# ChainSafe/lumenos

Hardware: AMD Instinct MI355X
Metric: prove_eval_seconds_16384x4096 (lower is better)
Workload: dtype u64; 1 GPU; Encode+Commit+InnerProduct(r,b)+QueryCols 16384x4096 LogN=14 L=12 K=2 rhoInv=2 queries=309; parallelism=1 GPU: the whole job resident in HBM

## Files before the change

### lumenos_amd/csrc/lm_keyswitch.hip

```cpp
#include <cstdlib>
#include <cstring>

#include "lm_ks_host.h"

static uint32_t ks_batch(const lumen_ctx *ctx) { return ctx->tune.ks_batch; }

__device__ __forceinline__ u32 bx_v(u128 A, u128 M, u64 y0, u64 y1, u64 m0, u64 m1) {
    const u128 D1 = A >= M ? A - M : M - A, D2 = 2 * M - A;
    if ((u64)(D1 >> 64) >= 8 && (u64)(D2 >> 64) >= 8) return A >= M ? 1u : 0u;
    double vf = 0.0;
    vf += (double)y0 / (double)m0;
    vf += (double)y1 / (double)m1;
    return (u32)(u64)vf;
}

__device__ __forceinline__ void pack_pair(u64 a, u64 b, u64 m0, u64 m1, u128 M, u64 &hi, u64 &lo) {
    u64 l1, h1, l2, h2;
    mul128(a, m1, l1, h1);
    mul128(b, m0, l2, h2);
    const u128 A = (((u128)h1 << 64) | l1) + (((u128)h2 << 64) | l2);
    const u32 v = bx_v(A, M, a, b, m0, m1);
    const u128 W = A + (v == 0 ? 2 * M : (v == 1 ? M : (u128)0));
    hi = (u64)(W >> LM_W_SPLIT), lo = (u64)W & ((1ull << LM_W_SPLIT) - 1);
}

__global__ __launch_bounds__(256) void k_pack_v(u64 *__restrict__ y, size_t poly_stride, uint32_t npoly,
                                                uint32_t ngroups, uint32_t group_limbs, uint32_t first_mod,
                                                uint32_t nlimbs_total, uint32_t logN, lm_mods mods) {
    const uint32_t N = 1u << logN;
    const size_t total = (size_t)npoly * ngroups * (N / 2), stride = (size_t)gridDim.x * blockDim.x;
    for (size_t g = (size_t)blockIdx.x * blockDim.x + threadIdx.x; g < total; g += stride) {
        const uint32_t i = (uint32_t)(g & (N / 2 - 1)) * 2;
        const uint32_t grp = (uint32_t)((g >> (logN - 1)) % ngroups), p = (uint32_t)((g >> (logN - 1)) / ngroups);
        const uint32_t l0 = grp * group_limbs;
        if (l0 + 1 >= nlimbs_total) continue;
        u64 *y0 = y + (size_t)p * poly_stride + (size_t)l0 * N + i;
        const ulonglong2 av = *reinterpret_cast<const ulonglong2 *>(y0);
        const ulonglong2 bv = *reinterpret_cast<const ulonglong2 *>(y0 + N);
        const u64 m0 = mods.m[first_mod + l0].q, m1 = mods.m[first_mod + l0 + 1].q;
        u64 Ml, Mh;
        mul128(m0, m1, Ml, Mh);
        const u128 M = ((u128)Mh << 64) | Ml;
        ulonglong2 hv, lv;
#pragma unroll
        for (int e = 0; e < 2; e++) {
            const u64 a = e ? av.y : av.x, b = e ? bv.y : bv.x;
            u64 hi, lo;
            pack_pair(a, b, m0, m1, M, hi, lo);
            if (e) hv.y = hi, lv.y = lo;
            else hv.x = hi, lv.x = lo;
        }
        *reinterpret_cast<ulonglong2 *>(y0) = hv;
        *reinterpret_cast<ulonglong2 *>(y0 + N) = lv;
    }
}

template <int LOGN>
__global__ LM_GEOM_BOUNDS(lm_geom_lds(LOGN)) void k_intt_pack(const u64 *__restrict__ acc, u64 *coef, uint32_t B,
                                                                  uint32_t L, uint32_t nf, lm_mods mods,
                                                                  lm_ninv_t yscale, const tw_t *__restrict__ tw_all) {
    extern __shared__ __attribute__((aligned(16))) u64 sm[];
    constexpr uint32_t N = 1u << LOGN;
    const uint32_t tid = threadIdx.x;
    if (blockIdx.x >= B * nf) {
        const uint32_t k = blockIdx.x - B * nf, l = 2 * nf + k / B, b = k % B;
        const u64 *p = acc + (((size_t)b * 2 + 1) * L + l) * N;
        u64 *o = coef + ((size_t)b * L + l) * N;
        const lm_qc q = lm_make_qc(mods.m[l]);
        const tw_t sc = yscale.t[l];
        auto ld = [&](uint32_t i0, u64 *v, int count) { lm_load_run(p, i0, v, count); };
        auto st = [&](uint32_t i, u64 v) { o[i] = lm_shoup_cs(v, sc, q.q, q.nq); };
        lm_ntt_inverse<LOGN>(sm, tw_all + (size_t)l * N, q, tid, ld, st);
        return;
    }
    const uint32_t d = blockIdx.x / B, b = blockIdx.x % B;
    const uint32_t l0 = 2 * d, l1 = l0 + 1;
    const u64 *c1 = acc + ((size_t)b * 2 + 1) * L * N;
    u64 *o0 = coef + ((size_t)b * L + l0) * N;
    const lm_qc q0 = lm_make_qc(mods.m[l0]);
    const tw_t s0 = yscale.t[l0];
    {
        const u64 *p = c1 + (size_t)l0 * N;
        auto ld = [&](uint32_t i0, u64 *v, int count) { lm_load_run(p, i0, v, count); };
        auto st = [&](uint32_t i, u64 v) { o0[i] = lm_shoup_cs(v, s0, q0.q, q0.nq); };
        lm_ntt_inverse<LOGN>(sm, tw_all + (size_t)l0 * N, q0, tid, ld, st);
    }
    __syncthreads();
    {
        const lm_qc q1 = lm_make_qc(mods.m[l1]);
        const tw_t s1 = yscale.t[l1];
        const u64 *p = c1 + (size_t)l1 * N;
        u64 Ml, Mh;
        mul128(q0.q, q1.q, Ml, Mh);
        auto uni = [](u64 x) {
            return (u64)(uint32_t)__builtin_amdgcn_readfirstlane((int)(uint32_t)x) |
                   (u64)(uint32_t)__builtin_amdgcn_readfirstlane((int)(uint32_t)(x >> 32)) << 32;
        };
        const u128 M = ((u128)uni(Mh) << 64) | uni(Ml);
        auto ld = [&](uint32_t i0, u64 *v, int count) { lm_load_run(p, i0, v, count); };
        constexpr int R_LAST = lm_pass_r(LOGN, 0), LOG_T0 = LOGN - R_LAST;
        constexpr int PF = (1 << R_LAST) * 5 / 8;
        struct pack_t {
            u64 *o0;
            const lm_qc &q0, &q1;
            tw_t s1;
            u128 M;
            u64 y0[PF];
            __device__ __forceinline__ void pre(uint32_t w) {
#pragma unroll
                for (int k = 0; k < PF; k++) y0[k] = o0[w + ((uint32_t)k << LOG_T0)];
            }
            __device__ __forceinline__ void operator()(uint32_t i, u64 v, int k) {
                const u64 y1 = lm_shoup_cs(v, s1, q1.q, q1.nq);
                uint32_t j = i;
                asm volatile("" : "+v"(j));
                const u64 a = k < PF ? y0[k < PF ? k : 0] : o0[j];
                u64 hi, lo;
                pack_pair(a, y1, q0.q, q1.q, M, hi, lo);
                o0[j] = hi, o0[j + N] = lo;
                if (k >= PF && (k & 1)) asm volatile("" ::: "memory");
            }
        } st{o0, q0, q1, s1, M, {}};
        uint32_t tid1 = tid;
        asm volatile("" : "+v"(tid1));
        lm_ntt_inverse<LOGN>(sm, tw_all + (size_t)l1 * N, q1, tid1, ld, st);
    }
}

template <int LOGN>
__global__ LM_GEOM_BOUNDS(lm_geom_fwd(LOGN)) void k_modup_ntt(const u64 *__restrict__ coef, const u64 *__restrict__ acc,
                                                    u64 *__restrict__ ext, const bx_t *__restrict__ bx,
                                                    uint32_t B, uint32_t L, uint32_t K, uint32_t beta,
                                                    const uint32_t *__restrict__ work, lm_mods mods,
                                                    const tw_t *__restrict__ tw_all) {
    extern __shared__ __attribute__((aligned(16))) u64 sm[];
    constexpr uint32_t N = 1u << LOGN;
    const uint32_t tid = threadIdx.x, LK = L + K;
    const uint32_t wk = work[blockIdx.x];
    const uint32_t b = wk & 0xFFFF, d = (wk >> 16) & 0xFF, t = wk >> 24;
    const bx_t c = bx[d * LK + t];
    u64 *o = ext + ks_ext_at(b, d, t, B, beta) * N;
    const lm_qc qc = lm_make_qc(mods.m[t]);
    const u64 *s0 = coef + ((size_t)b * L + d * K) * N;
    const u64 *s1 = c.ns == 2 ? s0 + N : s0;
    auto ld = [&](uint32_t i) { return bx_apply(c, s0[i], s1[i], qc); };
    auto out = [&](uint32_t j, u64 v0, u64 v1) {
        ulonglong2 y;
        y.x = v0, y.y = v1;
        *reinterpret_cast<ulonglong2 *>(o + j) = y;
    };
    if constexpr (LOGN == 14) {
        lm_w14_runs st{sm};
        auto after = [&](uint32_t i0, uint32_t) { lm_w14_linear_out(sm, tid, i0, out); };
        lm_ntt_forward_w14(sm, tw_all + (size_t)t * N, qc, tid, ld, st, after);
    } else {
        lm_lds_runs st{sm};
        auto after = [&](uint32_t, uint32_t) { lm_linear_out<LOGN>(sm, tid, out); };
        lm_ntt_forward<LOGN>(sm, tw_all + (size_t)t * N, qc, tid, ld, st, after);
    }
}

#ifndef LM_MAC_COLS
#define LM_MAC_COLS 4
#endif
#ifndef LM_MAC_VEC
#define LM_MAC_VEC 1
#endif
#ifndef LM_MAC_PREFETCH
#define LM_MAC_PREFETCH 1
#endif
template <int VEC>
struct mac_vec;
template <>
struct mac_vec<1> {
    u64 v[1];
    static __device__ __forceinline__ mac_vec load(const u64 *p) { return mac_vec{{*p}}; }
    static __device__ __forceinline__ mac_vec load_once(const u64 *p) { return mac_vec{{__builtin_nontemporal_load(p)}}; }
    __device__ __forceinline__ void store(u64 *p) const { *p = v[0]; }
};
template <>
struct mac_vec<2> {
    u64 v[2];
    static __device__ __forceinline__ mac_vec load(const u64 *p) {
        const ulonglong2 a = *reinterpret_cast<const ulonglong2 *>(p);
        return mac_vec{{a.x, a.y}};
    }
    static __device__ __forceinline__ mac_vec load_once(const u64 *p) {
        return mac_vec{{__builtin_nontemporal_load(p), __builtin_nontemporal_load(p + 1)}};
    }
    __device__ __forceinline__ void store(u64 *p) const {
        ulonglong2 a;
        a.x = v[0], a.y = v[1];
        *reinterpret_cast<ulonglong2 *>(p) = a;
    }
};
struct mac_acc {
    u64 a0, a1, a3;
    u32 c0, c1;
    __device__ __forceinline__ void clear() { a0 = a1 = a3 = 0, c0 = c1 = 0; }
    __device__ __forceinline__ void value(u64 &lo, u64 &hi) const {
        lo = a0 + (a1 << 32);
        hi = a3 + c0 + (a1 >> 32) + ((u64)c1 << 32) + (lo < a0 ? 1 : 0);
    }
};
__device__ __forceinline__ void mac2(mac_acc &p, mac_acc &q, u64 x, u64 k0, u64 k1) {
    const u32 x0 = (u32)x, x1 = (u32)(x >> 32);
#if LM_ASM_SHOUP
    asm("v_mad_u64_u32 %[pa0], s[98:99], %[x0], %[k00], %[pa0]\n\t"
// ... 282 lines not shown
    out->d_bxp = tb->d_bxp.get();
    out->d_pinv = tb->d_pinv.get();
    out->yscale = &tb->yscale;
    return 0;
}

int lm_launch_pack_v(lumen_ctx *ctx, u64 *y, size_t poly_stride, uint32_t npoly, uint32_t ngroups,
                     uint32_t group_limbs, uint32_t first_mod, uint32_t nlimbs_total) {
    hipLaunchKernelGGL(k_pack_v, dim3(2048), dim3(256), 0, ctx->stream, y, poly_stride, npoly, ngroups, group_limbs,
                       first_mod, nlimbs_total, ctx->logN, ctx->mods);
    LM_HIP(ctx, hipGetLastError());
    return 0;
}

namespace {

static int interleave_work_lists(lumen_ctx *ctx, const std::vector<std::vector<uint32_t>> &lists, size_t expect,
                                 const char *what, std::map<uint32_t, lm_dev<uint32_t>> &cache, uint32_t cache_key,
                                 const uint32_t **out) {
    std::vector<uint32_t> order;
    order.reserve(expect);
    std::vector<size_t> pos(8, 0);
    for (bool any = true; any;) {
        any = false;
        for (uint32_t x = 0; x < 8; x++)
            if (pos[x] < lists[x].size()) {
                order.push_back(lists[x][pos[x]++]);
                any = true;
            }
    }
    LM_CHECK(ctx, order.size() == expect, "%s work list is inconsistent", what);
    lm_dev<uint32_t> d;
    if (int rc = d.upload(ctx, order, "a key-switch work list")) return rc;
    *out = (cache[cache_key] = std::move(d)).get();
    return 0;
}

static int modup_work_list(lumen_ctx *ctx, KsTables *tb, uint32_t B, const uint32_t **out) {
    const uint32_t LM_MODUP_TGROUP = ctx->tune.modup_tgroup;
    LM_SHARED_LOCK(ctx);
    LM_CHECK(ctx, B >= 1 && B <= 65535 && tb->beta <= 255 && ctx->L + ctx->K <= 255,
             "key-switch batch of %u columns (beta %u) does not fit the packed work list", B, tb->beta);
    const uint32_t cache_key = B | (LM_MODUP_TGROUP << 16);
    auto it = tb->d_work.find(cache_key);
    if (it != tb->d_work.end()) {
        *out = it->second.get();
        return 0;
    }
    const uint32_t LK = ctx->L + ctx->K, beta = tb->beta;
    std::vector<std::vector<uint8_t>> need(beta);
    for (uint16_t pr : tb->pairs) need[pr & 0xFF].push_back((uint8_t)(pr >> 8));
    std::vector<std::vector<uint32_t>> lists(8);
    for (uint32_t x = 0; x < 8; x++)
        for (uint32_t t0 = 0; t0 < LK; t0 += LM_MODUP_TGROUP)
            for (uint32_t b = x; b < B; b += 8)
                for (uint32_t d = 0; d < beta; d++)
                    for (uint8_t t : need[d])
                        if (t >= t0 && t < t0 + LM_MODUP_TGROUP) lists[x].push_back(b | (d << 16) | ((uint32_t)t << 24));
    return interleave_work_lists(ctx, lists, (size_t)B * tb->pairs.size(), "extension", tb->d_work, cache_key, out);
}

static int moddown_work_list(lumen_ctx *ctx, KsTables *tb, uint32_t B, const uint32_t **out) {
    const uint32_t LM_MODDOWN_TGROUP = ctx->tune.moddown_tgroup;
    LM_SHARED_LOCK(ctx);
    LM_CHECK(ctx, B >= 1 && 2 * (uint64_t)B <= 65535, "key-switch batch of %u columns does not fit the packed work list", B);
    const uint32_t cache_key = B | (LM_MODDOWN_TGROUP << 17);
    auto it = tb->d_work_down.find(cache_key);
    if (it != tb->d_work_down.end()) {
        *out = it->second.get();
        return 0;
    }
    const uint32_t L = ctx->L;
    std::vector<std::vector<uint32_t>> lists(8);
    for (uint32_t x = 0; x < 8; x++)
        for (uint32_t t0 = 0; t0 < L; t0 += LM_MODDOWN_TGROUP)
            for (uint32_t pw = x; pw < 2 * B; pw += 8)
                for (uint32_t t = t0; t < std::min<uint32_t>(t0 + LM_MODDOWN_TGROUP, L); t++) lists[x].push_back(pw | (t << 16));
    return interleave_work_lists(ctx, lists, (size_t)2 * B * L, "ModDown", tb->d_work_down, cache_key, out);
}

static uint32_t ks_lanes(const lumen_ctx *ctx) {
    return ctx->tune.ks_lanes ? ctx->tune.ks_lanes : (ctx->logN <= 13 ? 2 : 1);
}
template <int LOGN>
static uint32_t intt_pack_slots(lumen_ctx *ctx) {
    static const uint32_t v = [&] {
        hipDeviceProp_t prop;
        int per_cu = 0;
        if (hipGetDeviceProperties(&prop, ctx->device) != hipSuccess) return 256u;
        (void)hipFuncSetAttribute(reinterpret_cast<const void *>(&k_intt_pack<LOGN>),
                                  hipFuncAttributeMaxDynamicSharedMemorySize, 160 * 1024);
        constexpr lm_geom g = lm_geom_lds(LOGN);
        if (hipOccupancyMaxActiveBlocksPerMultiprocessor(&per_cu, k_intt_pack<LOGN>, g.threads, g.lds) != hipSuccess || per_cu < 1) {
            per_cu = (int)std::max<size_t>(1, std::min<size_t>(160 * 1024 / g.lds, 2048 / g.threads));
        }
        (void)hipGetLastError();
        if (ctx->tune.debug)
            fprintf(stderr, "[lumenos_hip] k_intt_pack<%d>: %d workgroup(s) per CU, %d CUs\n", LOGN, per_cu,
                    prop.multiProcessorCount);
        return (uint32_t)prop.multiProcessorCount * (uint32_t)per_cu;
    }();
    return v;
}
static uint32_t ks_fused_digits(lumen_ctx *ctx, uint32_t B, uint32_t L) {
    const long forced = ctx->tune.ks_fused_digits;
    const uint32_t pairs = L / 2;
    if (forced >= 0) return std::min<uint32_t>((uint32_t)forced, pairs);
    uint32_t slots = 0;
    if (lm_for_logn(ctx, ctx->logN, [&](auto n) { return slots = intt_pack_slots<n>(ctx), 0; })) return 0;
    for (uint32_t nf = pairs; nf >= 1; nf--)
        if (((uint64_t)B * nf) % slots == 0) return nf;
    return 0;
}

struct LaneGuard {
    lumen_ctx *ctx;
    hipStream_t saved;
    LaneGuard(lumen_ctx *c, int lane) : ctx(c), saved(c->stream) {
        if (lane) ctx->stream = ctx->stream2;
    }
    ~LaneGuard() { ctx->stream = saved; }
};

static dim3 ks_mac_grid(const lumen_ctx *ctx, uint32_t B) {
    return dim3(((ctx->N / LM_MAC_VEC + 255) / 256) * (ctx->L + ctx->K) * ((B + LM_MAC_COLS - 1) / LM_MAC_COLS));
}

}

int rotate_accumulate(lumen_ctx *ctx, const u64 *acc, u64 *acc_out, uint32_t B, const lm_galois_key &gk,
                      KsTables *tb, const KsScratch &s) {
    const uint32_t N = ctx->N, L = ctx->L, K = ctx->K, beta = tb->beta;
    const uint32_t nf = K == 2 ? ks_fused_digits(ctx, B, L) : 0;
    if (nf) {
        const uint32_t grid = B * nf + B * (L - 2 * nf);
        lm_prof_scope ps(ctx, "ks_intt_c1", (uint64_t)B * L);
        if (int rc = lm_for_logn(ctx, ctx->logN, [&](auto n) {
                return lm_launch(ctx, k_intt_pack<n>, lm_geom_lds(n), grid, acc, s.coef, B, L, nf, ctx->mods, tb->yscale,
                                 ctx->sh->tw_inv.get());
            }))
            return rc;
    } else {
        if (int rc = lm_launch_ntt_strided(ctx, acc + (size_t)L * N, (size_t)2 * L * N, s.coef, (size_t)L * N, B,
                                           lm_map_q(L), true, "ks_intt_c1", &tb->yscale))
            return rc;
    }
    if (K == 2 && nf < beta) {
        lm_prof_scope ps(ctx, "ks_pack_v", (uint64_t)B);
        hipLaunchKernelGGL(k_pack_v, dim3(2048), dim3(256), 0, ctx->stream, s.coef + (size_t)2 * nf * N, (size_t)L * N,
                           B, beta - nf, K, 2 * nf, L - 2 * nf, ctx->logN, ctx->mods);
        LM_HIP(ctx, hipGetLastError());
    }
    {
        const uint64_t nb = (uint64_t)B * tb->pairs.size();
        const uint32_t *work = nullptr;
        if (int rc = modup_work_list(ctx, tb, B, &work)) return rc;
        lm_prof_scope ps(ctx, "ks_modup_ntt", nb);
        if (int rc = lm_for_logn(ctx, ctx->logN, [&](auto n) {
                return lm_launch(ctx, k_modup_ntt<n>, lm_geom_fwd(n), (uint32_t)nb, s.coef, acc, s.ext, tb->d_bx.get(), B, L, K, beta,
                                 work, ctx->mods, ctx->sh->tw_fwd.get());
            }))
            return rc;
    }
    {
        lm_prof_scope ps(ctx, "ks_mac", (uint64_t)B);
        hipLaunchKernelGGL(k_ks_mac, ks_mac_grid(ctx, B), dim3(256), 0, ctx->stream, s.ext, acc, gk.d_key.get(), s.u, B, L, K,
                           beta, ctx->logN, ctx->mods);
        LM_HIP(ctx, hipGetLastError());
    }
    {
        u64 *up = s.u + ks_u_at(0, L, B, L, K) * N;
        const size_t pstride = (size_t)K * N;
        if (int rc = lm_launch_ntt_strided(ctx, up, pstride, up, pstride, B * 2, lm_map_p(ctx), true, "ks_intt_p",
                                           &tb->yscale))
            return rc;
        if (K == 2) {
            lm_prof_scope ps(ctx, "ks_pack_v", (uint64_t)B);
            hipLaunchKernelGGL(k_pack_v, dim3(2048), dim3(256), 0, ctx->stream, up, pstride, B * 2, 1u, K, L, K,
                               ctx->logN, ctx->mods);
            LM_HIP(ctx, hipGetLastError());
        }
    }
    {
        const uint32_t *work_down = nullptr;
        if (int rc = moddown_work_list(ctx, tb, B, &work_down)) return rc;
        lm_prof_scope ps(ctx, "ks_moddown_ntt", (uint64_t)B * 2 * L);
        return lm_for_logn(ctx, ctx->logN, [&](auto n) {
            return lm_launch(ctx, k_moddown_ntt<n>, lm_geom_lds(n), B * 2 * L, s.u, acc, acc_out, tb->d_bxp.get(), tb->d_pinv.get(),
                             gk.d_index.get(), gk.d_inv_index.get(), work_down, B, L, K, ctx->mods, ctx->sh->tw_fwd.get());
        });
    }
}

namespace {

int inner_sum_batch(lumen_ctx *ctx, u64 *acc, uint32_t B, uint32_t n, KsTables *tb, const KsScratch &s) {
    uint64_t gal[64];
    const uint32_t cnt = lumen_inner_sum_galois_elements(ctx, n, gal);
    for (uint32_t r = 0; r < cnt; r++) {
        const lm_galois_key *gk;
        {
            LM_SHARED_LOCK(ctx);
            auto it = ctx->gkeys.find(gal[r]);
            LM_CHECK(ctx, it != ctx->gkeys.end(), "Galois key for element %llu not loaded",
                     (unsigned long long)gal[r]);
            gk = &it->second;
        }
        u64 *src = (r & 1) ? s.acc2 : acc, *dst = (r & 1) ? acc : s.acc2;
        if (int rc = rotate_accumulate(ctx, src, dst, B, *gk, tb, s)) return rc;
    }
    if (cnt & 1)
        LM_HIP(ctx, hipMemcpyAsync(acc, s.acc2, (size_t)B * 2 * ctx->L * ctx->N * 8, hipMemcpyDeviceToDevice,
                                   ctx->stream));
    return 0;
}

}

extern "C" int lumen_ks_mac_probe(lumen_ctx *ctx, uint32_t batch, const void *ext, const void *acc, const void *key,
                                  void *u, uint32_t reps, float *ms_per_launch) {
    LM_CHECK(nullptr, ctx && ms_per_launch, "lumen_ks_mac_probe: NULL argument");
// ... 122 lines not shown
```

### lumenos_amd/csrc/lm_ntt.hip

```cpp
#include "lm_ntt_dev.h"

template <int LOGN, bool INV>
constexpr lm_geom k_limb_ntt_geom = INV ? lm_geom_lds(LOGN) : lm_geom_fwd(LOGN);
template <int LOGN, bool INV>
__global__ LM_GEOM_BOUNDS((k_limb_ntt_geom<LOGN, INV>)) void k_limb_ntt(const u64 *src, size_t src_poly_stride, u64 *dst,
                                                   size_t dst_poly_stride, uint32_t npoly, lm_modmap map,
                                                   lm_mods mods, lm_ninv_t ninv,
                                                   const tw_t *__restrict__ tw_all) {
    extern __shared__ __attribute__((aligned(16))) u64 sm[];
    constexpr uint32_t N = 1u << LOGN;
    const uint32_t tid = threadIdx.x;
    const uint32_t limb = blockIdx.x / npoly, poly = blockIdx.x % npoly;
    const uint32_t mi = map.idx[limb];
    const lm_qc c = lm_make_qc(mods.m[mi]);
    const u64 *p = src + (size_t)poly * src_poly_stride + (size_t)limb * N;
    u64 *o = dst + (size_t)poly * dst_poly_stride + (size_t)limb * N;
    const tw_t *tw = tw_all + (size_t)mi * N;
    if (INV) {
        const tw_t ni = ninv.t[mi];
        auto st = [&](uint32_t i, u64 v) { o[i] = lm_shoup_cs(v, ni, c.q, c.nq); };
        auto ld = [&](uint32_t i0, u64 *v, int count) { lm_load_run(p, i0, v, count); };
        lm_ntt_inverse<LOGN>(sm, tw, c, tid, ld, st);
    } else {
        auto ld = [&](uint32_t i) { return p[i]; };
        auto st = [&](uint32_t i0, const u64 *v, int count) {
            u64 r[8];
#pragma unroll
            for (int k = 0; k < 8; k++)
                if (k < count) r[k] = lm_reduce_s(v[k], c.q, c.nq, c.qinv64);
            lm_store_run(o, i0, r, count);
        };
        if constexpr (LOGN == 14)
            lm_ntt_forward_w14(sm, tw, c, tid, ld, st);
        else
            lm_ntt_forward<LOGN>(sm, tw, c, tid, ld, st);
    }
}

static int launch_limb_ntt(lumen_ctx *ctx, uint32_t logn, bool inverse, uint32_t grid, const u64 *src,
                           size_t src_poly_stride, u64 *dst, size_t dst_poly_stride, uint32_t npoly,
                           const lm_modmap &map, const lm_mods &mods, const lm_ninv_t &ninv, const tw_t *tw) {
    return lm_for_logn(ctx, logn, [&](auto n) {
        if (inverse)
            return lm_launch(ctx, k_limb_ntt<n, true>, k_limb_ntt_geom<n, true>, grid, src, src_poly_stride, dst,
                             dst_poly_stride, npoly, map, mods, ninv, tw);
        return lm_launch(ctx, k_limb_ntt<n, false>, k_limb_ntt_geom<n, false>, grid, src, src_poly_stride, dst,
                         dst_poly_stride, npoly, map, mods, ninv, tw);
    });
}

int lm_launch_ntt_subring(lumen_ctx *ctx, uint32_t logn, const tw_t *tw, tw_t ninv_scale, const u64 *src,
                          size_t src_poly_stride, u64 *dst, size_t dst_poly_stride, uint32_t npoly,
                          uint32_t mod_idx, bool inverse, const mod_t *explicit_mod) {
    if (!npoly) return 0;
    lm_modmap map = lm_map_q(1);
    map.idx[0] = 0;
    lm_mods mods = ctx->mods;
    mods.m[0] = explicit_mod ? *explicit_mod : ctx->mods.m[mod_idx];
    lm_ninv_t ninv = lm_ninv_of(ctx);
    ninv.t[0] = ninv_scale;
    return launch_limb_ntt(ctx, logn, inverse, npoly, src, src_poly_stride, dst, dst_poly_stride, npoly, map, mods, ninv, tw);
}

int lm_launch_ntt_strided(lumen_ctx *ctx, const u64 *src, size_t src_poly_stride, u64 *dst,
                          size_t dst_poly_stride, uint32_t npoly, const lm_modmap &map, bool inverse,
                          const char *prof_name, const lm_ninv_t *inv_scale) {
    if (!npoly || !map.period) return 0;
    const lm_ninv_t ninv = inv_scale ? *inv_scale : lm_ninv_of(ctx);
    const uint64_t nblocks64 = (uint64_t)npoly * map.period;
    LM_CHECK(ctx, nblocks64 < (1ull << 31), "NTT grid too large: %llu", (unsigned long long)nblocks64);
    lm_prof_scope ps(ctx, prof_name ? prof_name : (inverse ? "limb_intt" : "limb_ntt"), nblocks64);
    return launch_limb_ntt(ctx, ctx->logN, inverse, (uint32_t)nblocks64, src, src_poly_stride, dst, dst_poly_stride, npoly,
                           map, ctx->mods, ninv, inverse ? ctx->sh->tw_inv.get() : ctx->sh->tw_fwd.get());
}

int lm_launch_ntt(lumen_ctx *ctx, u64 *d, uint32_t npoly, const lm_modmap &map, bool inverse) {
    const size_t stride = (size_t)map.period * ctx->N;
    return lm_launch_ntt_strided(ctx, d, stride, d, stride, npoly, map, inverse, nullptr, nullptr);
}

extern "C" int lumen_set_ntt(lumen_ctx *ctx, lumen_set *set, int inverse) {
    LM_CHECK(nullptr, ctx && set, "lumen_set_ntt: NULL argument");
    LM_ENTER(ctx);
    LM_FULL_WIDTH(ctx, set, "lumen_set_ntt");
    return lm_launch_ntt(ctx, set->d, set->count * 2, lm_map_q(set->nl), inverse != 0);
}
```

### lumenos_amd/csrc/lm_ntt_dev.h

```cpp
#pragma once
#include <cstring>
#include <type_traits>
#include <utility>

#include "lm_common.h"

#define LM_PAD(i) ((i) + ((i) >> 3))
template <int LOG_STRIDE>
__device__ __forceinline__ uint32_t lm_pad_at(uint32_t base, uint32_t pbase, int k) {
    if constexpr (LOG_STRIDE >= 3)
        return pbase + (uint32_t)k * ((1u << LOG_STRIDE) + (1u << (LOG_STRIDE - 3)));
    else
        return LM_PAD(base + ((uint32_t)k << LOG_STRIDE));
}
#define LM_MAX_PASSES 8

struct lm_ninv_t {
    tw_t t[LM_MAX_LIMBS];
};

__host__ __device__ constexpr int lm_ilog2(int x) { return x <= 1 ? 0 : 1 + lm_ilog2(x >> 1); }
__host__ __device__ constexpr size_t lm_lds_for(uint32_t n) { return (size_t)(n + (n >> 3) + 2) * sizeof(u64); }
struct lm_geom {
    int threads;
// ... 648 lines not shown
#ifndef LM_INV_TW_PREFETCH
#define LM_INV_TW_PREFETCH 1
#endif
template <int LOGN, int R, int LT>
__device__ __forceinline__ void lm_inv_mid(u64 *s, const tw_t *tw, const lm_qc &c, uint32_t tid) {
    using D = lm_deal<LOGN, R>;
    if (!D::valid(tid)) return;
    constexpr bool UW = LT >= 6;
    lm_inv_twset<R, UW, false> T[2];
    T[0].load(tw, LOGN, LT, D::local(tid, 0) >> LT);
#pragma unroll
    for (uint32_t m = 0; m < D::reps; m++) {
        const uint32_t w = D::local(tid, m);
        const uint32_t blk = w >> LT, off = w & ((1u << LT) - 1);
        const uint32_t base = (blk << (LT + R)) + off;
        u64 e[1 << R];
        const uint32_t pb = LM_PAD(base);
#pragma unroll
        for (int k = 0; k < (1 << R); k++) e[k] = s[lm_pad_at<LT>(base, pb, k)];
        if (LM_INV_TW_PREFETCH && m + 1 < D::reps) T[(m + 1) & 1].load(tw, LOGN, LT, D::local(tid, m + 1) >> LT);
        if (!LM_INV_TW_PREFETCH && m) T[0].load(tw, LOGN, LT, blk);
        lm_inv_stages<R, UW, false, false>(e, T[LM_INV_TW_PREFETCH ? (m & 1) : 0], c);
#pragma unroll
        for (int k = 0; k < (1 << R); k++) s[lm_pad_at<LT>(base, pb, k)] = e[k];
    }
}

template <class S, class = void>
struct lm_has_slot : std::false_type {};
template <class S>
struct lm_has_slot<S, std::void_t<decltype(std::declval<S &>()(0u, (u64)0, 0))>> : std::true_type {};

template <int LOGN, int R, class Storer>
__device__ __forceinline__ void lm_inv_last(const u64 *s, const tw_t *tw, const lm_qc &c, uint32_t tid, Storer &st) {
    constexpr uint32_t log_t0 = LOGN - R, items = 1u << log_t0, NT = lm_nthreads(LOGN);
    constexpr uint32_t reps = items / NT ? items / NT : 1;
    lm_inv_twset<R, true, false> T;
    T.load(tw, LOGN, log_t0, 0);
#pragma unroll 1
    for (uint32_t m = 0; m < reps; m++) {
        const uint32_t w = tid + m * NT;
        if (items < NT && w >= items) break;
        u64 e[1 << R];
#pragma unroll
        for (int k = 0; k < (1 << R); k++) e[k] = s[lm_pad_at<log_t0>(w, LM_PAD(w), k)];
        if constexpr (lm_has_pre<Storer>::value) st.pre(w);
        lm_inv_stages<R, true, true, false>(e, T, c);
#pragma unroll
        for (int k = 0; k < (1 << R); k++) {
            if constexpr (lm_has_slot<Storer>::value)
                st(w + ((uint32_t)k << log_t0), e[k], k);
            else
                st(w + ((uint32_t)k << log_t0), e[k]);
        }
    }
}

template <int LOGN, int P, int LT, class Loader, class Storer>
__device__ __forceinline__ void lm_inv_rec(u64 *sm, const tw_t *tw, const lm_qc &c, uint32_t tid, Loader &ld,
                                           Storer &st) {
    constexpr int NP = lm_npasses(LOGN), R = lm_pass_r(LOGN, NP - 1 - P);
    constexpr bool cross = lm_cross_r(LOGN) > 0;
    if constexpr (P == 0)
        lm_inv_first<LOGN, R>(sm, tw, c, tid, ld);
    else if constexpr (P == NP - 1)
        lm_inv_last<LOGN, R>(sm, tw, c, tid, st);
    else
        lm_inv_mid<LOGN, R, LT>(sm, tw, c, tid);
    if constexpr (P + 1 < NP) {
        if constexpr (P + 2 == NP && cross)
            __syncthreads();
        else
            lm_wave_sync();
        lm_inv_rec<LOGN, P + 1, LT + R>(sm, tw, c, tid, ld, st);
    }
}
template <int LOGN, class Loader, class Storer>
__device__ __forceinline__ void lm_ntt_inverse(u64 *sm, const tw_t *tw, const lm_qc &c, uint32_t tid, Loader &ld,
                                               Storer &st) {
    static_assert(lm_npasses(LOGN) >= 2, "a transform needs a loading and a storing pass");
    lm_inv_rec<LOGN, 0, 0>(sm, tw, c, tid, ld, st);
}

__device__ __forceinline__ void lm_load_run(const u64 *p, uint32_t i0, u64 *v, int count) {
    if (count == 2) {
        const ulonglong2 a = *reinterpret_cast<const ulonglong2 *>(p + i0);
        v[0] = a.x, v[1] = a.y;
    } else {
#pragma unroll
        for (int k = 0; k < 8; k += 2) {
            if (k < count) {
                const ulonglong2 a = *reinterpret_cast<const ulonglong2 *>(p + i0 + k);
                v[k] = a.x, v[k + 1] = a.y;
            }
        }
    }
}
struct lm_lds_runs {
    u64 *sm;
    __device__ __forceinline__ void operator()(uint32_t i0, const u64 *v, int count) const {
#pragma unroll
        for (int k = 0; k < 8; k++)
            if (k < count) sm[LM_PAD(i0 + k)] = v[k];
    }
};
template <int LOGN, class F>
__device__ __forceinline__ void lm_linear_out(const u64 *sm, uint32_t tid, F f) {
    constexpr uint32_t NW = lm_nthreads(LOGN) / 64, BLK = (1u << LOGN) / NW, IT = BLK / 128 ? BLK / 128 : 1;
    const uint32_t wave = tid >> 6, lane = tid & 63;
    lm_wave_sync();
#pragma unroll
    for (uint32_t k = 0; k < IT; k++) {
        const uint32_t j = wave * BLK + 2 * lane + k * 128;
        if (BLK >= 128 || 2 * lane < BLK) f(j, sm[LM_PAD(j)], sm[LM_PAD(j + 1)]);
    }
}

__device__ __forceinline__ void lm_store_run(u64 *p, uint32_t i0, const u64 *v, int count) {
#pragma unroll
    for (int k = 0; k < 8; k += 2) {
        if (k < count) {
            ulonglong2 a;
            a.x = v[k], a.y = v[k + 1];
            *reinterpret_cast<ulonglong2 *>(p + i0 + k) = a;
        }
    }
}
```

### lumenos_amd/csrc/lm_rescale.hip

```cpp
#include "lm_ntt_dev.h"

struct rescale_consts {
    u64 half;
    u64 half_mod[LM_MAX_LIMBS];
    tw_t qlinv[LM_MAX_LIMBS];
};

template <int LOGN>
__global__ LM_GEOM_BOUNDS(lm_geom_lds(LOGN)) void k_rescale_last(const u64 *__restrict__ src, size_t src_poly_stride,
                                                       uint32_t last, u64 *__restrict__ tbuf, mod_t md,
                                                       tw_t ninv, u64 half, const tw_t *__restrict__ tw) {
    extern __shared__ __attribute__((aligned(16))) u64 sm[];
    constexpr uint32_t N = 1u << LOGN;
    const uint32_t tid = threadIdx.x;
    const lm_qc c = lm_make_qc(md);
    const u64 *p = src + (size_t)blockIdx.x * src_poly_stride + (size_t)last * N;
    u64 *o = tbuf + (size_t)blockIdx.x * N;
    auto ld = [&](uint32_t i0, u64 *v, int count) { lm_load_run(p, i0, v, count); };
    auto st = [&](uint32_t i, u64 v) { o[i] = lm_addmod(lm_shoup_cs(v, ninv, c.q, c.nq), half, c.q); };
    lm_ntt_inverse<LOGN>(sm, tw, c, tid, ld, st);
}

template <int LOGN>
__global__ LM_GEOM_BOUNDS(lm_geom_lds(LOGN)) void k_rescale_limb(const u64 *src, size_t src_poly_stride, u64 *dst,
                                                       size_t dst_poly_stride, const u64 *__restrict__ tbuf,
                                                       uint32_t npoly, lm_mods mods, rescale_consts rc,
                                                       const tw_t *__restrict__ tw_all) {
    extern __shared__ __attribute__((aligned(16))) u64 sm[];
    constexpr uint32_t N = 1u << LOGN;
    const uint32_t tid = threadIdx.x;
    const uint32_t limb = blockIdx.x / npoly, poly = blockIdx.x % npoly;
    const lm_qc c = lm_make_qc(mods.m[limb]);
    const u64 hm = rc.half_mod[limb];
    const tw_t qlinv = rc.qlinv[limb];
    const u64 *t = tbuf + (size_t)poly * N;
    const u64 *cin = src + (size_t)poly * src_poly_stride + (size_t)limb * N;
    u64 *o = dst + (size_t)poly * dst_poly_stride + (size_t)limb * N;
    auto ld = [&](uint32_t i) { return lm_submod(lm_reduce_s(t[i], c.q, c.nq, c.qinv64), hm, c.q); };
    auto st = [&](uint32_t i0, const u64 *v, int count) {
        u64 cv[8], r[8];
        lm_load_run(cin, i0, cv, count);
#pragma unroll
        for (int k = 0; k < 8; k++)
            if (k < count) r[k] = lm_shoup_cs(lm_submod(cv[k], lm_reduce_s(v[k], c.q, c.nq, c.qinv64), c.q), qlinv, c.q, c.nq);
        lm_store_run(o, i0, r, count);
    };
    lm_ntt_forward<LOGN>(sm, tw_all + (size_t)limb * N, c, tid, ld, st);
}

struct rs_step_t {
    u64 k;
    u64 pad;
    tw_t inv;
};
struct rs_half_t {
    u64 h[LM_MAX_LIMBS];
};
struct RescaleTables {
    lm_dev<rs_step_t> d_steps;
    rs_half_t half;
};

static int get_rescale_tables(lumen_ctx *ctx, RescaleTables **out) {
    LM_SHARED_LOCK(ctx);
    auto it = ctx->ext.find("rescale_tables");
    if (it != ctx->ext.end()) {
        *out = static_cast<RescaleTables *>(it->second.get());
        return 0;
    }
    auto sp = std::make_shared<RescaleTables>();
    std::vector<rs_step_t> steps((size_t)LM_MAX_LIMBS * LM_MAX_LIMBS);
    memset(steps.data(), 0, steps.size() * sizeof(rs_step_t));
    for (uint32_t l = 0; l < LM_MAX_LIMBS; l++) {
        const uint64_t ql = ctx->mod[l < ctx->L ? l : 0], half = (ql - 1) >> 1;
        sp->half.h[l] = half;
        for (uint32_t j = 0; j < l && l < ctx->L; j++) {
            const uint64_t qj = ctx->mod[j];
            rs_step_t &e = steps[(size_t)l * LM_MAX_LIMBS + j];
            const uint64_t M = ql / qj + 1;
            if (M > 16) return 2;
            e.k = half + M * qj;
            e.inv = h_tw(h_invmod(ql % qj, qj), qj);
        }
    }
    if (int rc = sp->d_steps.upload(ctx, steps, "the rescale tables")) return rc;
    ctx->ext["rescale_tables"] = sp;
    *out = sp.get();
    return 0;
}

__global__ __launch_bounds__(256) void k_rescale_coef(const u64 *__restrict__ coef, size_t src_poly_stride,
                                                      u64 *__restrict__ dst, size_t dst_poly_stride, uint32_t nl,
                                                      uint32_t target, uint32_t logN, size_t total, lm_mods mods,
                                                      const rs_step_t *__restrict__ steps, rs_half_t half) {
    const size_t idx = (size_t)blockIdx.x * blockDim.x + threadIdx.x;
    if (idx >= total) return;
    const size_t poly = idx >> logN, i = idx & (((size_t)1 << logN) - 1);
    const u64 *p = coef + poly * src_poly_stride + i;
    u64 c[LM_MAX_LIMBS];
#pragma unroll
    for (int j = 0; j < LM_MAX_LIMBS; j++) c[j] = (uint32_t)j < nl ? p[(size_t)j << logN] : 0;
#pragma unroll
    for (int l = LM_MAX_LIMBS - 1; l >= 1; l--) {
        if ((uint32_t)l < nl && (uint32_t)l >= target) {
            const u64 ql = mods.m[l].q;
            u64 t = lm_csub(lm_csub(c[l], 2 * ql), ql);
            t = lm_addmod(t, half.h[l], ql);
#pragma unroll
            for (int j = 0; j < l; j++) {
                const rs_step_t e = steps[l * LM_MAX_LIMBS + j];
                c[j] = lm_shoup3<true>(c[j] + e.k - t, e.inv.w, e.inv.wp, 0 - mods.m[j].q);
            }
        }
    }
    u64 *o = dst + poly * dst_poly_stride + i;
#pragma unroll
    for (int j = 0; j < LM_MAX_LIMBS; j++)
        if ((uint32_t)j < target) {
            const u64 qj = mods.m[j].q;
            o[(size_t)j << logN] = lm_csub(lm_csub(c[j], 2 * qj), qj);
        }
}

static int rescale_polys_coef(lumen_ctx *ctx, const u64 *src, uint32_t nl, u64 *dst, uint32_t target, uint32_t npoly,
                              u64 *work) {
    RescaleTables *tb = nullptr;
    if (int rc = get_rescale_tables(ctx, &tb)) return rc;
    const uint32_t N = ctx->N;
    if (int rc = lm_launch_ntt_strided(ctx, src, (size_t)nl * N, work, (size_t)nl * N, npoly, lm_map_q(nl), true,
                                       "rescale_intt", nullptr))
        return rc;
    {
        lm_prof_scope ps(ctx, "rescale_coef", npoly);
        const size_t total = (size_t)npoly * N;
        hipLaunchKernelGGL(k_rescale_coef, dim3((uint32_t)((total + 255) / 256)), dim3(256), 0, ctx->stream, work,
                           (size_t)nl * N, dst, (size_t)target * N, nl, target, ctx->logN, total, ctx->mods,
                           tb->d_steps.get(), tb->half);
        LM_HIP(ctx, hipGetLastError());
    }
    return lm_launch_ntt_strided(ctx, dst, (size_t)target * N, dst, (size_t)target * N, npoly, lm_map_q(target), false,
                                 "rescale_ntt", nullptr);
}

template <int LOGN>
static int rescale_polys_t(lumen_ctx *ctx, const u64 *src, uint32_t nl, u64 *dst, uint32_t target,
                           uint32_t npoly, u64 *work, u64 *tbuf) {
    if (work && (uint64_t)(nl + target + 1) * (nl - target) / 2 > (uint64_t)nl + target) {
        const int rc = rescale_polys_coef(ctx, src, nl, dst, target, npoly, work);
        if (rc != 2) return rc;
    }
    const uint32_t N = ctx->N;
    const u64 *cur = src;
    for (uint32_t cur_nl = nl; cur_nl > target; cur_nl--) {
        const uint32_t last = cur_nl - 1;
        const bool final_step = cur_nl - 1 == target;
        u64 *out = final_step ? dst : work;
        const size_t out_stride = (size_t)(final_step ? target : nl) * N;
        rescale_consts rc;
        const uint64_t ql = ctx->mod[last];
        rc.half = (ql - 1) >> 1;
        for (uint32_t i = 0; i < LM_MAX_LIMBS; i++) {
            const uint64_t qi = ctx->mod[i < last ? i : 0];
            rc.half_mod[i] = rc.half % qi;
            rc.qlinv[i] = h_tw(h_invmod(ql % qi, qi), qi);
        }
        {
            lm_prof_scope ps(ctx, "rescale_last_intt", npoly);
            if (int e = lm_launch(ctx, k_rescale_last<LOGN>, lm_geom_lds(LOGN), npoly, cur, (size_t)nl * N, last, tbuf,
                                  ctx->mods.m[last], ctx->ninv[last], (u64)rc.half, ctx->sh->tw_inv.get() + (size_t)last * N))
                return e;
        }
        {
            lm_prof_scope ps(ctx, "rescale_limb_ntt", (uint64_t)npoly * last);
            if (int e = lm_launch(ctx, k_rescale_limb<LOGN>, lm_geom_lds(LOGN), npoly * last, cur, (size_t)nl * N, out,
                                  out_stride, tbuf, npoly, ctx->mods, rc, ctx->sh->tw_fwd.get()))
                return e;
        }
        cur = work;
    }
    return 0;
}

int lm_rescale_polys(lumen_ctx *ctx, const u64 *src, uint32_t nl, u64 *dst, uint32_t target,
                     uint32_t npoly, u64 *work, u64 *tbuf) {
    return lm_for_logn(ctx, ctx->logN, [&](auto n) { return rescale_polys_t<n>(ctx, src, nl, dst, target, npoly, work, tbuf); });
}

extern "C" int lumen_rescale(lumen_ctx *ctx, const lumen_set *in, uint32_t target_limbs, lumen_set **out) {
    LM_CHECK(nullptr, ctx && in && out, "lumen_rescale: NULL argument");
    LM_ENTER(ctx);
    LM_FULL_WIDTH(ctx, in, "lumen_rescale");
    LM_CHECK(ctx, target_limbs >= 1 && target_limbs <= in->nl, "target_limbs %u out of range [1,%u]",
             target_limbs, in->nl);
    lumen_set *o = nullptr;
    if (int rc = lumen_set_create(ctx, in->count, target_limbs, &o)) return rc;
    lm_set_guard og(ctx, o);
    const uint32_t N = ctx->N, nl = in->nl;
    const size_t in_ctw = (size_t)2 * nl * N, out_ctw = (size_t)2 * target_limbs * N;
    if (target_limbs == nl) {
        if (in->words)
            LM_HIP(ctx, hipMemcpyAsync(o->d, in->d, in->words * sizeof(u64), hipMemcpyDeviceToDevice, ctx->stream));
        *out = og.release();
        return 0;
    }
    uint32_t chunk = (uint32_t)std::max<size_t>(1, ((size_t)2 << 30) / (in_ctw * sizeof(u64)));
    if (chunk >= 128) chunk -= chunk % 128;
    chunk = std::min(chunk, std::max(in->count, 1u));
    u64 *work = nullptr;
    if (nl - target_limbs > 1) {
        work = (u64 *)lm_scratch(ctx, "rescale_work", (size_t)chunk * in_ctw * sizeof(u64));
        if (!work) return 1;
    }
    u64 *tbuf = (u64 *)lm_scratch(ctx, "rescale_t", (size_t)chunk * 2 * N * sizeof(u64));
    if (!tbuf) return 1;
    for (uint32_t first = 0; first < in->count; first += chunk) {
        const uint32_t n = std::min(chunk, in->count - first);
        if (int rc = lm_rescale_polys(ctx, in->d + (size_t)first * in_ctw, nl, o->d + (size_t)first * out_ctw,
                                      target_limbs, n * 2, work, tbuf))
            return rc;
    }
    *out = og.release();
    return 0;
}
```

Measured before the change: 1.802 s.

## Add register-heavy wave-local inverse NTT path for LogN=14 kernels

Introduces a specialised inverse NTT for N=2^14 in which each thread holds 32 coefficients in registers. The first stages run wave-locally with only wave syncs, a single block-wide LDS exchange follows, and a fused last-five-stages routine finishes the transform. The inverse-NTT, intt_pack and rescale kernels switch to this path with a new launch geometry (lm_geom_inv) that uses half the LDS. The pack storer now prefetches the partner limb in chunks, and the fused-digit count heuristic changes to balance load per CU instead of divisibility by slot count. In exchange there is higher register pressure, a more complex code path, and inline asm readfirstlane with s_nop hazards.

```diff
diff --git a/lumenos_amd/csrc/lm_keyswitch.hip b/lumenos_amd/csrc/lm_keyswitch.hip
--- a/lumenos_amd/csrc/lm_keyswitch.hip
+++ b/lumenos_amd/csrc/lm_keyswitch.hip
@@ -1,3 +1,4 @@
+#include <atomic>
 #include <cstdlib>
 #include <cstring>
 
@@ -55,25 +56,43 @@
     }
 }
 
+#ifndef LM_W14_PACK_CHUNK
+#define LM_W14_PACK_CHUNK 4
+#endif
+#ifndef LM_W14_PACK_AHEAD
+#define LM_W14_PACK_AHEAD 0
+#endif
 template <int LOGN>
-__global__ LM_GEOM_BOUNDS(lm_geom_lds(LOGN)) void k_intt_pack(const u64 *__restrict__ acc, u64 *coef, uint32_t B,
+__global__ LM_GEOM_BOUNDS(lm_geom_inv(LOGN)) void k_intt_pack(const u64 *__restrict__ acc, u64 *coef, uint32_t B,
                                                                   uint32_t L, uint32_t nf, lm_mods mods,
                                                                   lm_ninv_t yscale, const tw_t *__restrict__ tw_all) {
     extern __shared__ __attribute__((aligned(16))) u64 sm[];
     constexpr uint32_t N = 1u << LOGN;
     const uint32_t tid = threadIdx.x;
+    auto wg = [](uint32_t x) {
+        if constexpr (LOGN == 14) {
+            uint32_t r;
+            asm("s_nop 1\n\tv_readfirstlane_b32 %0, %1\n\ts_nop 4" : "=s"(r) : "v"(x));
+            return r;
+        } else {
+            return x;
+        }
+    };
     if (blockIdx.x >= B * nf) {
-        const uint32_t k = blockIdx.x - B * nf, l = 2 * nf + k / B, b = k % B;
+        const uint32_t k = blockIdx.x - B * nf, l = 2 * nf + wg(k / B), b = wg(k % B);
         const u64 *p = acc + (((size_t)b * 2 + 1) * L + l) * N;
         u64 *o = coef + ((size_t)b * L + l) * N;
         const lm_qc q = lm_make_qc(mods.m[l]);
         const tw_t sc = yscale.t[l];
         auto ld = [&](uint32_t i0, u64 *v, int count) { lm_load_run(p, i0, v, count); };
         auto st = [&](uint32_t i, u64 v) { o[i] = lm_shoup_cs(v, sc, q.q, q.nq); };
-        lm_ntt_inverse<LOGN>(sm, tw_all + (size_t)l * N, q, tid, ld, st);
+        if constexpr (LOGN == 14)
+            lm_ntt_inverse_w14(sm, tw_all + (size_t)l * N, q, tid, ld, st);
+        else
+            lm_ntt_inverse<LOGN>(sm, tw_all + (size_t)l * N, q, tid, ld, st);
         return;
     }
-    const uint32_t d = blockIdx.x / B, b = blockIdx.x % B;
+    const uint32_t d = wg(blockIdx.x / B), b = wg(blockIdx.x % B);
     const uint32_t l0 = 2 * d, l1 = l0 + 1;
     const u64 *c1 = acc + ((size_t)b * 2 + 1) * L * N;
     u64 *o0 = coef + ((size_t)b * L + l0) * N;
@@ -83,7 +102,10 @@
         const u64 *p = c1 + (size_t)l0 * N;
         auto ld = [&](uint32_t i0, u64 *v, int count) { lm_load_run(p, i0, v, count); };
         auto st = [&](uint32_t i, u64 v) { o0[i] = lm_shoup_cs(v, s0, q0.q, q0.nq); };
-        lm_ntt_inverse<LOGN>(sm, tw_all + (size_t)l0 * N, q0, tid, ld, st);
+        if constexpr (LOGN == 14)
+            lm_ntt_inverse_w14(sm, tw_all + (size_t)l0 * N, q0, tid, ld, st);
+        else
+            lm_ntt_inverse<LOGN>(sm, tw_all + (size_t)l0 * N, q0, tid, ld, st);
     }
     __syncthreads();
     {
@@ -123,7 +145,29 @@
         } st{o0, q0, q1, s1, M, {}};
         uint32_t tid1 = tid;
         asm volatile("" : "+v"(tid1));
-        lm_ntt_inverse<LOGN>(sm, tw_all + (size_t)l1 * N, q1, tid1, ld, st);
+        if constexpr (LOGN == 14) {
+            struct pack14_t {
+                enum { chunk = LM_W14_PACK_CHUNK, ahead = LM_W14_PACK_AHEAD };
+                u64 *o0;
+                const lm_qc &q0, &q1;
+                tw_t s1;
+                u128 M;
+                u64 y0[2 * chunk];
+                __device__ __forceinline__ void pre(uint32_t i, int par) {
+#pragma unroll
+                    for (int k = 0; k < chunk; k++) y0[par * chunk + k] = o0[i + ((uint32_t)k << 9)];
+                }
+                __device__ __forceinline__ void operator()(uint32_t i, u64 v, int slot) {
+                    const u64 y1 = lm_shoup_cs(v, s1, q1.q, q1.nq);
+                    u64 hi, lo;
+                    pack_pair(y0[slot], y1, q0.q, q1.q, M, hi, lo);
+                    o0[i] = hi, o0[i + N] = lo;
+                }
+            } st14{o0, q0, q1, s1, M, {}};
+            lm_ntt_inverse_w14(sm, tw_all + (size_t)l1 * N, q1, tid1, ld, st14);
+        } else {
+            lm_ntt_inverse<LOGN>(sm, tw_all + (size_t)l1 * N, q1, tid1, ld, st);
+        }
     }
 }
 
@@ -572,15 +616,18 @@
 static uint32_t ks_lanes(const lumen_ctx *ctx) {
     return ctx->tune.ks_lanes ? ctx->tune.ks_lanes : (ctx->logN <= 13 ? 2 : 1);
 }
+struct intt_pack_dev {
+    uint32_t cus, per_cu;
+};
 template <int LOGN>
-static uint32_t intt_pack_slots(lumen_ctx *ctx) {
-    static const uint32_t v = [&] {
+static intt_pack_dev intt_pack_slots(lumen_ctx *ctx) {
+    static const intt_pack_dev v = [&] {
         hipDeviceProp_t prop;
         int per_cu = 0;
-        if (hipGetDeviceProperties(&prop, ctx->device) != hipSuccess) return 256u;
+        if (hipGetDeviceProperties(&prop, ctx->device) != hipSuccess) return intt_pack_dev{256u, 1u};
         (void)hipFuncSetAttribute(reinterpret_cast<const void *>(&k_intt_pack<LOGN>),
                                   hipFuncAttributeMaxDynamicSharedMemorySize, 160 * 1024);
-        constexpr lm_geom g = lm_geom_lds(LOGN);
+        constexpr lm_geom g = lm_geom_inv(LOGN);
         if (hipOccupancyMaxActiveBlocksPerMultiprocessor(&per_cu, k_intt_pack<LOGN>, g.threads, g.lds) != hipSuccess || per_cu < 1) {
             per_cu = (int)std::max<size_t>(1, std::min<size_t>(160 * 1024 / g.lds, 2048 / g.threads));
         }
@@ -588,19 +635,38 @@
         if (ctx->tune.debug)
             fprintf(stderr, "[lumenos_hip] k_intt_pack<%d>: %d workgroup(s) per CU, %d CUs\n", LOGN, per_cu,
                     prop.multiProcessorCount);
-        return (uint32_t)prop.multiProcessorCount * (uint32_t)per_cu;
+        return intt_pack_dev{(uint32_t)std::max(1, prop.multiProcessorCount), (uint32_t)per_cu};
     }();
     return v;
+}
+static uint32_t ks_fused_digits_rule(uint32_t B, uint32_t L, uint32_t cus, uint32_t per_cu) {
+    const uint64_t total = (uint64_t)B * L;
+    if (total <= (uint64_t)cus * per_cu) return 0;
+    const uint64_t share = (total + cus - 1) / cus;
+    for (uint32_t nf = L / 2; nf >= 1; nf--)
+        if (2 * (((uint64_t)B * nf + cus - 1) / cus) <= share) return nf;
+    return 0;
 }
 static uint32_t ks_fused_digits(lumen_ctx *ctx, uint32_t B, uint32_t L) {
     const long forced = ctx->tune.ks_fused_digits;
     const uint32_t pairs = L / 2;
-    if (forced >= 0) return std::min<uint32_t>((uint32_t)forced, pairs);
-    uint32_t slots = 0;
-    if (lm_for_logn(ctx, ctx->logN, [&](auto n) { return slots = intt_pack_slots<n>(ctx), 0; })) return 0;
-    for (uint32_t nf = pairs; nf >= 1; nf--)
-        if (((uint64_t)B * nf) % slots == 0) return nf;
-    return 0;
+    uint32_t nf = 0;
+    if (forced >= 0) {
+        nf = std::min<uint32_t>((uint32_t)forced, pairs);
+    } else {
+        intt_pack_dev dev{};
+        if (lm_for_logn(ctx, ctx->logN, [&](auto n) { return dev = intt_pack_slots<n>(ctx), 0; })) return 0;
+        nf = ks_fused_digits_rule(B, L, dev.cus, dev.per_cu);
+    }
+    if (ctx->tune.debug) {
+        static std::atomic<uint64_t> said{~0ull};
+        const uint64_t key = (uint64_t)B << 32 | (uint64_t)L << 8 | nf;
+        if (said.exchange(key) != key) {
+            fprintf(stderr, "[lumenos_hip] ks_fused_digits: B = %u, L = %u -> %u of %u digits packed in k_intt_pack%s\n", B, L,
+                    nf, pairs, forced >= 0 ? " (forced)" : "");
+        }
+    }
+    return nf;
 }
 
 struct LaneGuard {
@@ -626,7 +692,7 @@
         const uint32_t grid = B * nf + B * (L - 2 * nf);
         lm_prof_scope ps(ctx, "ks_intt_c1", (uint64_t)B * L);
         if (int rc = lm_for_logn(ctx, ctx->logN, [&](auto n) {
-                return lm_launch(ctx, k_intt_pack<n>, lm_geom_lds(n), grid, acc, s.coef, B, L, nf, ctx->mods, tb->yscale,
+                return lm_launch(ctx, k_intt_pack<n>, lm_geom_inv(n), grid, acc, s.coef, B, L, nf, ctx->mods, tb->yscale,
                                  ctx->sh->tw_inv.get());
             }))
             return rc;
diff --git a/lumenos_amd/csrc/lm_ntt.hip b/lumenos_amd/csrc/lm_ntt.hip
--- a/lumenos_amd/csrc/lm_ntt.hip
+++ b/lumenos_amd/csrc/lm_ntt.hip
@@ -1,7 +1,7 @@
 #include "lm_ntt_dev.h"
 
 template <int LOGN, bool INV>
-constexpr lm_geom k_limb_ntt_geom = INV ? lm_geom_lds(LOGN) : lm_geom_fwd(LOGN);
+constexpr lm_geom k_limb_ntt_geom = INV ? lm_geom_inv(LOGN) : lm_geom_fwd(LOGN);
 template <int LOGN, bool INV>
 __global__ LM_GEOM_BOUNDS((k_limb_ntt_geom<LOGN, INV>)) void k_limb_ntt(const u64 *src, size_t src_poly_stride, u64 *dst,
                                                    size_t dst_poly_stride, uint32_t npoly, lm_modmap map,
@@ -20,7 +20,10 @@
         const tw_t ni = ninv.t[mi];
         auto st = [&](uint32_t i, u64 v) { o[i] = lm_shoup_cs(v, ni, c.q, c.nq); };
         auto ld = [&](uint32_t i0, u64 *v, int count) { lm_load_run(p, i0, v, count); };
-        lm_ntt_inverse<LOGN>(sm, tw, c, tid, ld, st);
+        if constexpr (LOGN == 14)
+            lm_ntt_inverse_w14(sm, tw, c, tid, ld, st);
+        else
+            lm_ntt_inverse<LOGN>(sm, tw, c, tid, ld, st);
     } else {
         auto ld = [&](uint32_t i) { return p[i]; };
         auto st = [&](uint32_t i0, const u64 *v, int count) {
diff --git a/lumenos_amd/csrc/lm_ntt_dev.h b/lumenos_amd/csrc/lm_ntt_dev.h
--- a/lumenos_amd/csrc/lm_ntt_dev.h
+++ b/lumenos_amd/csrc/lm_ntt_dev.h
@@ -754,6 +754,154 @@
     lm_inv_rec<LOGN, 0, 0>(sm, tw, c, tid, ld, st);
 }
 
+template <class S, class = void>
+struct lm_has_pre2 : std::false_type {};
+template <class S>
+struct lm_has_pre2<S, std::void_t<decltype(std::declval<S &>().pre(0u, 0))>> : std::true_type {};
+
+__device__ __forceinline__ void lm_inv_stages_last5(u64 *e, const tw_t *tw, const lm_qc &c) {
+    constexpr int R = 5, RED = 3;
+    static_assert(3 * (1 << RED) <= 3 * 14 + 8 && 3 * (1 << (R - RED)) <= 3 * 14 + 8,
+                  "3q * 2^stages must stay below the (3 * logN + 8) * q < 2^64 the context guarantees");
+#pragma unroll
+    for (int st = 0; st < R; st++) {
+        const int half = 1 << st, span = half << 1, CH = half < 8 ? half : 8;
+        const u64 C = c.q3 << (st >= RED ? st - RED : st);
+#pragma unroll
+        for (int g = 0; g < ((1 << R) / span); g++) {
+            const tw_t W = lm_tw_load<true>(tw, (1u << (R - 1 - st)) + g);
+#pragma unroll
+            for (int k0 = 0; k0 < half; k0 += CH) {
+                u64 dif[8];
+#pragma unroll
+                for (int k = 0; k < CH; k++) {
+                    u64 &x = e[g * span + k0 + k], &y = e[g * span + k0 + k + half];
+                    dif[k] = x + C - y;
+                    x = x + y;
+                }
+#pragma unroll
+                for (int k = 0; k < CH; k++) e[g * span + k0 + k + half] = lm_shoup3<true>(dif[k], W.w, W.wp, c.nq);
+            }
+        }
+        if (st == RED - 1) {
+#pragma unroll
+            for (int i = 0; i < (1 << R); i++) {
+                const int j = i & ((1 << RED) - 1);
+                if (j >= (1 << RED) / 2) continue;
+                const int k = j == 0 ? RED : RED - 1 - lm_ilog2(j);
+                if (k >= 3) {
+                    e[i] = lm_shoup3<true>(e[i], 1ull, c.qinv64, c.nq);
+                } else {
+#pragma unroll
+                    for (int q = k - 1; q >= 0; q--) e[i] = lm_csub(e[i], c.q3 << q);
+                }
+            }
+        }
+    }
+}
+
+template <class Loader, class Storer>
+__device__ __forceinline__ void lm_ntt_inverse_w14(u64 *sm, const tw_t *tw, const lm_qc &c, uint32_t tid, Loader &ld,
+                                                   Storer &st) {
+    const uint32_t w = tid >> 6, l = tid & 63;
+    u64 e[32];
+    const uint32_t p1 = LM_PAD(tid), p2 = LM_PAD((w << 10) | l);
+    const uint32_t p3 = LM_PAD((w << 10) | ((l >> 3) << 6) | (l & 7)), p4 = LM_PAD((w << 10) | (l << 3));
+#pragma unroll
+    for (int m = 0; m < 4; m++) {
+        LM_W14_FENCE();
+        const uint32_t i0 = (w << 11) | ((uint32_t)m << 9) | (l << 3);
+        lm_inv_twset<3, false, true> T;
+        T.load(tw, 14, 0, i0 >> 3);
+        ld(i0, e + 8 * m, 8);
+        lm_inv_stages<3, false, false, true>(e + 8 * m, T, c);
+    }
+#pragma unroll
+    for (int h = 0; h < 2; h++) {
+        lm_wave_sync();
+#pragma unroll
+        for (int r = 16 * h; r < 16 * h + 16; r++)
+            sm[lm_w14_at(p4, (uint32_t)(((r >> 3) & 1) << 9 | (r & 7)))] = e[r];
+        lm_wave_sync();
+#pragma unroll
+        for (int r = 16 * h; r < 16 * h + 16; r++)
+            e[r] = sm[lm_w14_at(p3, (uint32_t)(((r >> 3) & 1) << 9 | (r & 7) << 3))];
+    }
+#pragma unroll
+    for (int m = 0; m < 4; m++) {
+        LM_W14_FENCE();
+        lm_inv_twset<3, false, false> T;
+        T.load(tw, 14, 3, (w << 5) | ((uint32_t)m << 3) | (l >> 3));
+        lm_inv_stages<3, false, false, false>(e + 8 * m, T, c);
+    }
+#pragma unroll
+    for (int h = 0; h < 2; h++) {
+        lm_wave_sync();
+#pragma unroll
+        for (int r = 16 * h; r < 16 * h + 16; r++)
+            sm[lm_w14_at(p3, (uint32_t)(((r >> 3) & 1) << 9 | (r & 7) << 3))] = e[r];
+        lm_wave_sync();
+#pragma unroll
+        for (int r = 16 * h; r < 16 * h + 16; r++) e[r] = sm[lm_w14_at(p2, (uint32_t)(r & 15) << 6)];
+    }
+#pragma unroll
+    for (int m = 0; m < 4; m++) {
+        LM_W14_FENCE();
+        lm_inv_twset<3, true, false> T;
+        T.load(tw, 14, 6, (w << 2) | (uint32_t)m);
+        lm_inv_stages<3, true, false, false>(e + 8 * m, T, c);
+    }
+    u64 t0[16];
+#pragma unroll
+    for (int h = 0; h < 2; h++) {
+        if (h) __syncthreads();
+#pragma unroll
+        for (int r = 16 * h; r < 16 * h + 16; r++) sm[lm_w14_at(p2, (uint32_t)(r & 15) << 6)] = e[r];
+        __syncthreads();
+        int n = 0;
+#pragma unroll
+        for (int r = 0; r < 32; r++)
+            if (((r >> 1) & 1) == h) {
+                const u64 v = sm[lm_w14_at(p1, (uint32_t)((r >> 2) << 10 | (r & 1) << 9))];
+                if (h)
+                    e[r] = v;
+                else
+                    t0[n] = v;
+                n++;
+            }
+    }
+    {
+        int n = 0;
+#pragma unroll
+        for (int r = 0; r < 32; r++)
+            if (((r >> 1) & 1) == 0) e[r] = t0[n++];
+    }
+    LM_W14_FENCE();
+    lm_inv_stages_last5(e, tw, c);
+    LM_W14_FENCE();
+    if constexpr (lm_has_pre2<Storer>::value) {
+        constexpr int CH = Storer::chunk;
+        constexpr bool AHEAD = Storer::ahead != 0;
+        static_assert(32 % CH == 0, "chunks of the last pass");
+        st.pre(tid, 0);
+#pragma unroll
+        for (int r0 = 0; r0 < 32; r0 += CH) {
+            const int par = AHEAD ? (r0 / CH) & 1 : 0;
+            if (AHEAD && r0 && r0 + CH < 32) st.pre(((uint32_t)(r0 + CH) << 9) | tid, par ^ 1);
+#pragma unroll
+            for (int k = 0; k < CH; k++) st(((uint32_t)(r0 + k) << 9) | tid, e[r0 + k], par * CH + k);
+            LM_W14_FENCE();
+            if ((!AHEAD || !r0) && r0 + CH < 32) st.pre(((uint32_t)(r0 + CH) << 9) | tid, AHEAD ? par ^ 1 : 0);
+        }
+    } else {
+#pragma unroll
+        for (int r = 0; r < 32; r++) st(((uint32_t)r << 9) | tid, e[r]);
+    }
+}
+__host__ __device__ constexpr lm_geom lm_geom_inv(int logN) {
+    return logN == 14 ? lm_geom{LM_W14_THREADS, 4, lm_lds_for(1u << 13)} : lm_geom_lds(logN);
+}
+
 __device__ __forceinline__ void lm_load_run(const u64 *p, uint32_t i0, u64 *v, int count) {
     if (count == 2) {
         const ulonglong2 a = *reinterpret_cast<const ulonglong2 *>(p + i0);
diff --git a/lumenos_amd/csrc/lm_rescale.hip b/lumenos_amd/csrc/lm_rescale.hip
--- a/lumenos_amd/csrc/lm_rescale.hip
+++ b/lumenos_amd/csrc/lm_rescale.hip
@@ -7,7 +7,7 @@
 };
 
 template <int LOGN>
-__global__ LM_GEOM_BOUNDS(lm_geom_lds(LOGN)) void k_rescale_last(const u64 *__restrict__ src, size_t src_poly_stride,
+__global__ LM_GEOM_BOUNDS(lm_geom_inv(LOGN)) void k_rescale_last(const u64 *__restrict__ src, size_t src_poly_stride,
                                                        uint32_t last, u64 *__restrict__ tbuf, mod_t md,
                                                        tw_t ninv, u64 half, const tw_t *__restrict__ tw) {
     extern __shared__ __attribute__((aligned(16))) u64 sm[];
@@ -18,7 +18,10 @@
     u64 *o = tbuf + (size_t)blockIdx.x * N;
     auto ld = [&](uint32_t i0, u64 *v, int count) { lm_load_run(p, i0, v, count); };
     auto st = [&](uint32_t i, u64 v) { o[i] = lm_addmod(lm_shoup_cs(v, ninv, c.q, c.nq), half, c.q); };
-    lm_ntt_inverse<LOGN>(sm, tw, c, tid, ld, st);
+    if constexpr (LOGN == 14)
+        lm_ntt_inverse_w14(sm, tw, c, tid, ld, st);
+    else
+        lm_ntt_inverse<LOGN>(sm, tw, c, tid, ld, st);
 }
 
 template <int LOGN>
@@ -166,7 +169,7 @@
         }
         {
             lm_prof_scope ps(ctx, "rescale_last_intt", npoly);
-            if (int e = lm_launch(ctx, k_rescale_last<LOGN>, lm_geom_lds(LOGN), npoly, cur, (size_t)nl * N, last, tbuf,
+            if (int e = lm_launch(ctx, k_rescale_last<LOGN>, lm_geom_inv(LOGN), npoly, cur, (size_t)nl * N, last, tbuf,
                                   ctx->mods.m[last], ctx->ninv[last], (u64)rc.half, ctx->sh->tw_inv.get() + (size_t)last * N))
                 return e;
         }
```

Result: no change. 1.800 s, median of 2 (-0.1%).
